# chongminggao/CIRS-codes

Measured on AMD Instinct MI355X. Metric: simulator env-steps/s (collect + PPO update in the timed region), KuaishouEnv, higher is better.
Workload: dtype f32 (policy/tracker; rollout on the fp32 MFMA, PPO head products fp32-accurate from two fp16 pieces per operand (3 f16 MFMAs per product), fp32 accumulate) + f64 (env rewards, GAE)

## Files before the change

cirs-codes_amd/csrc/ppo.hip:

```cpp
#include "internal.h"
#include "optim.h"
#include "bf16x6.h"
#include "small_gemm.h"
#include "permutation.h"
#include "policy_kernels.h"

namespace cirs {
typedef float f32x4 __attribute__((ext_vector_type(4)));


constexpr int kBwdWaves = 4;
__host__ __device__ inline int n_row_blocks_of(int n_pad) { return (n_pad / kTileM + kBwdWaves - 1) / kBwdWaves; }
__host__ __device__ inline size_t dwa_slab_stride(int I) { return (((size_t)I * 64 + I) + 3) & ~(size_t)3; }
__host__ __device__ inline int n_dwa_slabs_of(int n_pad) { return n_row_blocks_of(n_pad); }

struct PpoLayout {
    long w1, b1, w2, b2, wa, ba, wc, bc, total, trunk;
};
__host__ __device__ inline PpoLayout ppo_layout(int I, int S) {
    PpoLayout L;
    L.w1 = 0; L.b1 = L.w1 + (long)kH * S; L.w2 = L.b1 + kH; L.b2 = L.w2 + (long)kH * kH;
    L.trunk = L.b2 + kH;
    L.wa = L.trunk; L.ba = L.wa + (long)I * kH; L.wc = L.ba + I; L.bc = L.wc + kH; L.total = L.bc + 1;
    return L;
// ... 527 lines not shown
constexpr int kTStride = 36;
constexpr int kRSize = kTileN * kH + 2 * kTileN;
constexpr int kRowB = 144, kColB = 80;
constexpr int kRPlaneB = kTileN * kRowB, kCPlaneB = kH * kColB;
constexpr int kWBufB = 3 * kRPlaneB + 3 * kCPlaneB;

#ifdef CIRS_HEAD_PROF
__device__ unsigned long long g_step_prof[64];
#define CIRS_PSTAMP(COND, K) do { if ((COND) && threadIdx.x == 0) g_step_prof[K] = __builtin_amdgcn_s_memtime(); } while (0)
#else
#define CIRS_PSTAMP(COND, K) do { } while (0)
#endif
#ifdef CIRS_HEAD_PROF
__device__ unsigned long long g_head_prof[64];
#define CIRS_HSTAMP(K) do { if (blockIdx.x == 0 && blockIdx.y == 0 && threadIdx.x == 0 && it == 2) g_head_prof[K] = __builtin_amdgcn_s_memtime(); } while (0)
#define CIRS_TSTAMP(B, K) do { if ((int)blockIdx.x == (B) && threadIdx.x == 0) g_head_prof[K] = __builtin_amdgcn_s_memtime(); } while (0)
#define CIRS_SSTAMP(K) do { if (blockIdx.x == 0 && blockIdx.y == 0 && threadIdx.x == 0) g_head_prof[K] = __builtin_amdgcn_s_memtime(); } while (0)
#else
#define CIRS_HSTAMP(K) do { } while (0)
#define CIRS_TSTAMP(B, K) do { } while (0)
#define CIRS_SSTAMP(K) do { } while (0)
#endif
template <bool kZout>
__global__ __launch_bounds__(256, 2) void head_stats_kernel(int I, int mb, int n_pad, int tiles_per_chunk,
                                                            const uint4* __restrict__ planes, const float* __restrict__ ba,
                                                            const uint4* __restrict__ h2z, ActorPartialView pv,
                                                            const int32_t* __restrict__ act_rows, float* __restrict__ za_out,
                                                            float4* __restrict__ zslab) {
    __shared__ __attribute__((aligned(16))) unsigned char sW[2][3 * kRPlaneB];
    __shared__ __attribute__((aligned(16))) float sB[2][kTileN];
    const int tid = threadIdx.x;
    CIRS_SSTAMP(40);
    const int lane = tid & 63, wv = tid >> 6;
    const int hi = lane >> 5, lo = lane & 31;
// ... 119 lines not shown
            run_s = run_s * fa + osum * fb;
            run_t = run_t * fa + ot * fb;
            run_m = mn;
        }
    }
    if (hi == 0) {
        const size_t po = (size_t)chunk * n_pad + jr;
        pv.score[po] = run_t; pv.m[po] = run_m; pv.s[po] = run_s;
    }
    if (za_have) za_out[jr] = za_val;
}



struct HeadMergeArgs { cirs_ppo_cfg cfg; cirs_ppo_batch b; const int32_t* idx; int mb_norm, n_schunks; ActorPartialView pv; };
template <bool kEnt, bool kMerge, bool kZin>
__global__ __launch_bounds__(kBwdWaves * 64, 1) void head_bwd_fused_kernel(int I, int mb, int n_pad, int tiles_per_chunk,
                                                                         const uint4* __restrict__ planes,
                                                                         const float* __restrict__ ba, MbView v,
                                                                         float* __restrict__ dwap, HeadMergeArgs ma) {
    constexpr int kThreads = kBwdWaves * 64;
    static_assert(kThreads == 256, "the plane staging maps one 16-byte unit per thread and plane");
    constexpr int kCOff = kZin ? 0 : 3 * kRPlaneB;
    __shared__ __attribute__((aligned(16))) unsigned char sW[2][kCOff + 3 * kCPlaneB];
    __shared__ __attribute__((aligned(16))) float sB[2][kTileN];
    __shared__ __attribute__((aligned(16))) float sT[kBwdWaves][kTileN * kTStride];
    __shared__ __attribute__((aligned(16))) float sR[2][kBwdWaves][kRSize];
    const int tid = threadIdx.x;
    CIRS_SSTAMP(30);
    if (blockIdx.x == 0 && blockIdx.y == 0) {
        v.sync[tid] = 0;
        if (tid < kSyncInts - 256) v.sync[256 + tid] = 0;
    }
    const int lane = tid & 63, wv = tid >> 6;
    const int hi = lane >> 5, lo = lane & 31;
    const int row0 = (blockIdx.y * kBwdWaves + wv) * kTileM;
    const bool wave_ok = row0 < n_pad;
    const int chunk = blockIdx.x;
    if (chunk * tiles_per_chunk * kTileN >= I) return;
    const int jr = wave_ok ? row0 + lo : 0;
    const float kLog2e = 1.4426950408889634f, kLn2 = 0.6931471805599453f;
    const int act = v.act[jr];
    HPl hz[4];
    HPl hb[2][2];
    {
        const size_t tb = (size_t)((wave_ok ? row0 : 0) >> 5) * 12 * 64 + lane;
        const uint4* zp = v.h2z + tb;
        const uint4* bp = v.h2b + tb;
        if (!kZin) {
#pragma unroll
            for (int s4 = 0; s4 < 4; ++s4) {
                HPL_SET(hz[s4], zp[(3 * s4) * 64], zp[(3 * s4 + 2) * 64]);
            }
        }
#pragma unroll
        for (int c = 0; c < 2; ++c)
#pragma unroll
            for (int t = 0; t < 2; ++t) {
                HPL_SET(hb[c][t], bp[(3 * (2 * c + t)) * 64], bp[(3 * (2 * c + t) + 2) * 64]);
            }
    }
    const bool row_ok = wave_ok && jr < mb;
    f32x16 dh0, dh1;
#pragma unroll
    for (int r = 0; r < 16; ++r) { dh0[r] = 0.f; dh1[r] = 0.f; }
    float ent = 0.f;
    const float eps = 1.1920928955078125e-7f;
    const float kLogEps = -15.942385152878742f, kLog1mEps = -1.1920929665620834e-7f;
    if (!wave_ok) {
        for (int q = lane; q < kRSize; q += 64) { sR[0][wv][q] = 0.f; sR[1][wv][q] = 0.f; }
    }

    const int first_tile = chunk * tiles_per_chunk * kTileN;
    const int n_tiles = max(0, min(tiles_per_chunk, (I - first_tile + kTileN - 1) / kTileN));
    const int dst_r = (tid >> 3) * kRowB + (tid & 7) * 16;
    const int dst_c = kCOff + (tid >> 2) * kColB + (tid & 3) * 16;
    uint4 gr0, gr2, gc0, gc2;
    float gb = 0.f;
#define CIRS_ISSUE(TILE0)                                                                                  \
    do {                                                                                                   \
        const uint4* src_ = planes + (size_t)((TILE0) / kTileN) * kPlaneTileU4 + tid;                      \
        if (!kZin) { gr0 = src_[0]; gr2 = src_[512]; }                                                     \
        gc0 = src_[768]; gc2 = src_[1280];                                                                 \
        if (!kZin && tid < kTileN) gb = ((TILE0) + tid) < I ? kScZ * ba[(TILE0) + tid] : 0.f;    \
    } while (0)
#define CIRS_COMMIT(BUF)                                                                                   \
    do {                                                                                                   \
        unsigned char* base_ = sW[BUF];                                                                    \
        if (!kZin) {                                                                                       \
            *reinterpret_cast<uint4*>(base_ + dst_r) = gr0;                                                \
            *reinterpret_cast<uint4*>(base_ + 2 * kRPlaneB + dst_r) = gr2;                                 \
        }                                                                                                  \
        *reinterpret_cast<uint4*>(base_ + dst_c) = gc0;                                                    \
        \
        *reinterpret_cast<uint4*>(base_ + 2 * kCPlaneB + dst_c) = gc2;                                     \
        if (!kZin && tid < kTileN) sB[BUF][tid] = gb;                                                      \
    } while (0)
    const float4* zsl = v.zslab + ((size_t)(first_tile / kTileN) * (n_pad / kTileM) + (wave_ok ? row0 / kTileM : 0)) * kZTileF4 + lane;
    const size_t zstep = (size_t)(n_pad / kTileM) * kZTileF4;
    float4 zn[4];
    if (kZin) {
#pragma unroll
        for (int q = 0; q < 4; ++q) zn[q] = zsl[q * 64];
    }
    if (n_tiles > 0) CIRS_ISSUE(first_tile);
    float lse, c_logp, c_ent, h_ent;
    if (!kMerge) {
        lse = v.lse[jr]; c_logp = v.c_logp[jr]; c_ent = kEnt ? v.c_ent[jr] : 0.f; h_ent = kEnt ? v.h_ent[jr] : 0.f;
    } else {
        const bool real = wave_ok && jr < mb;
        const int jc = real ? jr : 0;
        const float za = v.za[jc], adv = v.adv[jc], lpo = v.adv[n_pad + jc], ret = v.adv[2 * (size_t)n_pad + jc], vs = v.adv[3 * (size_t)n_pad + jc],
                    val = v.value[jc];
        const float red0 = v.red[0], red1 = v.red[1];
        const int nsc = ma.n_schunks;
        const float* __restrict__ pm_ = ma.pv.m + jc;
        const float* __restrict__ ps_ = ma.pv.s + jc;
        const float* __restrict__ pt_ = ma.pv.score + jc;
        float M = -INFINITY, ssum = 0.f, tsum = 0.f;
        const bool need_t = kEnt || blockIdx.x == 0;
// ... 34 lines not shown
        ssum += __shfl_xor(ssum, 32, CIRS_WAVE);
        tsum += __shfl_xor(tsum, 32, CIRS_WAVE);
        const float lse_r = M + __logf(ssum);
        const RowTerms rt = ppo_row_terms(ma.cfg, za, lse_r, tsum / ssum, lpo, adv, red0, red1, val, vs, ret, 1.0f / (float)ma.mb_norm);
        lse = real ? lse_r : 1e30f;
        c_logp = real ? rt.c_logp : 0.f;
        c_ent = (kEnt && real) ? rt.c_ent : 0.f;
        h_ent = (kEnt && real) ? rt.h_ent : 0.f;
        if (blockIdx.x == 0 && hi == 0 && wave_ok) {
            v.dvalue[jr] = real ? rt.dvalue : 0.f;
            v.clip_row[jr] = real ? rt.clip_row : 0.f;
            v.vf_row[jr] = real ? rt.vf_row : 0.f;
            v.h_ent[jr] = real ? rt.h_ent : 0.f;
        }
    }
    float dz_scale = 1.0f, dz_inv = 1.0f;
    __shared__ float s_cmax[kBwdWaves];
    {
        const float cm = wave_max_f32_dpp(fabsf(c_logp) + 16.0f * fabsf(c_ent));
        if (lane == 0) s_cmax[wv] = cm;
    }
    CIRS_SSTAMP(31);
    if (n_tiles > 0) CIRS_COMMIT(0);
    __syncthreads();
    {
        float cm = s_cmax[0];
#pragma unroll
        for (int q = 1; q < kBwdWaves; ++q) cm = fmaxf(cm, s_cmax[q]);
        int ex = 0;
        if (cm > 0.f) { (void)frexpf(cm, &ex); ex = max(ex, -80); dz_scale = ldexpf(1.0f, 14 - ex); dz_inv = ldexpf(1.0f, ex - 14); }
        c_logp *= dz_scale; c_ent *= dz_scale;
    }
    const float nlse2 = -(lse * kLog2e), ncl = -c_logp;
    CIRS_SSTAMP(32);
    float* slab = dwap + (size_t)blockIdx.y * dwa_slab_stride(I);
    constexpr int kRedQ = (kTileN * kH / 4) / kThreads;
    const float dw_unscale = dz_inv * (1.0f / kScH2), dh_unscale = dz_inv * (1.0f / kScWa);
    struct RedRegs { f32x4 t[kRedQ][kBwdWaves]; float b[kBwdWaves]; };
    auto reduce_load = [&](int rb, RedRegs& rg) {
#pragma unroll
        for (int q = 0; q < kRedQ; ++q)
#pragma unroll
            for (int w2 = 0; w2 < kBwdWaves; ++w2) rg.t[q][w2] = reinterpret_cast<const f32x4*>(sR[rb][w2])[tid + kThreads * q];
        if (wv == 0) {
#pragma unroll
            for (int w2 = 0; w2 < kBwdWaves; ++w2) rg.b[w2] = sR[rb][w2][kTileN * kH + lo] + sR[rb][w2][kTileN * kH + kTileN + lo];
        }
    };
    auto reduce_store = [&](const RedRegs& rg, int t0) {
        const bool full = t0 + kTileN <= I;
#pragma unroll
        for (int q = 0; q < kRedQ; ++q) {
            const int f = tid + kThreads * q;
            f32x4 t = rg.t[q][0];
#pragma unroll
            for (int w2 = 1; w2 < kBwdWaves; ++w2) t += rg.t[q][w2];
            t *= dw_unscale;
            if (full || t0 + (f >> 4) < I) *reinterpret_cast<f32x4*>(slab + (size_t)t0 * kH + 4 * f) = t;
        }
        if (wv == 0) {
            float t = rg.b[0];
#pragma unroll
            for (int w2 = 1; w2 < kBwdWaves; ++w2) t += rg.b[w2];
            if (hi == 0 && (full || t0 + lo < I)) slab[(size_t)I * kH + t0 + lo] = t * dz_inv;
        }
    };
    auto reduce_tile = [&](int rb, int t0) { RedRegs rg; reduce_load(rb, rg); reduce_store(rg, t0); };
    for (int it = 0; it < n_tiles; ++it) {
        const int buf = it & 1;
        const int tile0 = first_tile + it * kTileN;
        CIRS_HSTAMP(0);
        if (it + 1 < n_tiles) CIRS_ISSUE(tile0 + kTileN);
        f32x16 dw0, dw1;
        float db = 0.f;
        if (!wave_ok) {
            if (it + 1 < n_tiles) CIRS_COMMIT(buf ^ 1);
            if (it > 0) reduce_tile(buf ^ 1, tile0 - kTileN);
        }
        if (wave_ok) {
            const unsigned char* tw = sW[buf];
            HPl cb[2][2];
            f32x16 acc;
            RedRegs rg;
            if (kZin) {
#pragma unroll
                for (int q = 0; q < 4; ++q) { acc[4 * q] = zn[q].x; acc[4 * q + 1] = zn[q].y; acc[4 * q + 2] = zn[q].z; acc[4 * q + 3] = zn[q].w; }
                const float4* zp = zsl + (size_t)min(it + 1, n_tiles - 1) * zstep;
#pragma unroll
                for (int q = 0; q < 4; ++q) zn[q] = zp[q * 64];
                CIRS_HSTAMP(1);
            } else {
                HPl za[4];
#pragma unroll
                for (int s4 = 0; s4 < 4; ++s4) {
                    const unsigned char* ap = tw + lo * kRowB + (16 * s4 + 8 * hi) * 2;
                    HPL_SET(za[s4], *reinterpret_cast<const uint4*>(ap), *reinterpret_cast<const uint4*>(ap + 2 * kRPlaneB));
                }
                f32x16 acc1, acc2;
#pragma unroll
                for (int r = 0; r < 16; ++r) { acc[r] = sB[buf][acc_row(r, hi)]; acc1[r] = 0.f; acc2[r] = 0.f; }
                CIRS_HSTAMP(1);
                hmfma_split2(za[0], hz[0], za[1], hz[1], acc, acc1, acc2);
                if (it > 0) reduce_load(buf ^ 1, rg);
                hmfma_split2(za[2], hz[2], za[3], hz[3], acc, acc1, acc2);
#pragma unroll
                for (int r = 0; r < 16; ++r) acc[r] += acc1[r] + acc2[r];
                if (it > 0) reduce_store(rg, tile0 - kTileN);
            }
#pragma unroll
            for (int t = 0; t < 2; ++t)
#pragma unroll
                for (int c = 0; c < 2; ++c) {
                    const unsigned char* bp = tw + kCOff + (32 * c + lo) * kColB + (16 * t + 8 * hi) * 2;
                    HPL_SET(cb[c][t], *reinterpret_cast<const uint4*>(bp), *reinterpret_cast<const uint4*>(bp + 2 * kCPlaneB));
                }
            CIRS_HSTAMP(2);
            float* tt = sT[wv];
            f32x16 tk;
            float pmax = 0.f, elo = 0.f;
            f32x2_b elo2 = {0.f, 0.f};
            const float kTEps = -23.0f;
            const bool last_tile = tile0 + kTileN > I;
#pragma unroll
            for (int r = 0; r < 16; r += 2) {
                const float t0 = __builtin_fmaf(acc[r], kLog2e * kScZi, nlse2), t1 = __builtin_fmaf(acc[r + 1], kLog2e * kScZi, nlse2);
                const float p0 = __builtin_amdgcn_exp2f(t0), p1 = __builtin_amdgcn_exp2f(t1);
                tk[r] = t0; tk[r + 1] = t1;
                pmax = __builtin_fmaxf(__builtin_fmaxf(pmax, p0), p1);
                if (!last_tile) {
                    const f32x2_b d2 = f32x2_b{kTEps, kTEps} - f32x2_b{t0, t1};
                    const f32x2_b w2 = {__builtin_fmaxf(d2.x, 0.f), __builtin_fmaxf(d2.y, 0.f)};
                    elo2 = f32x2_b{p0, p1} * w2 + elo2;
                }
                if (kEnt) {
                    acc[r] = __builtin_fmaf(c_ent * p0, __builtin_fmaf(t0, kLn2, h_ent), ncl * p0);
                    acc[r + 1] = __builtin_fmaf(c_ent * p1, __builtin_fmaf(t1, kLn2, h_ent), ncl * p1);
                } else {
// ... 14 lines not shown
                }
            }
            ent -= kLn2 * (elo + (elo2.x + elo2.y));
            CIRS_HSTAMP(3);
#pragma unroll
            for (int r = 0; r < 16; ++r) tt[acc_row(r, hi) * kTStride + lo] = acc[r];
            if (__any(row_ok && pmax > 1.0f - eps)) {
#pragma unroll
                for (int r = 0; r < 16; ++r) {
                    const float p = __builtin_amdgcn_exp2f(tk[r]);
                    const bool ok = row_ok && (!last_tile || tile0 + acc_row(r, hi) < I);
                    ent -= (ok && p > 1.0f - eps) ? p * (kLog1mEps - tk[r] * kLn2) : 0.f;
                }
            }
            CIRS_HSTAMP(4);
            __builtin_amdgcn_fence(__ATOMIC_RELEASE, "wavefront");
            __builtin_amdgcn_wave_barrier();
            __builtin_amdgcn_fence(__ATOMIC_ACQUIRE, "wavefront");
            f32x16 dzt;
#pragma unroll
            for (int g = 0; g < 4; ++g) {
                const float4 t4 = *reinterpret_cast<const float4*>(&tt[lo * kTStride + 8 * g + 4 * hi]);
                dzt[4 * g] = t4.x; dzt[4 * g + 1] = t4.y; dzt[4 * g + 2] = t4.z; dzt[4 * g + 3] = t4.w;
            }
            if (it + 1 < n_tiles) CIRS_COMMIT(buf ^ 1);
            {
                const HPl a0 = hsplit8(acc, 0), a1 = hsplit8(acc, 8);
                if (kZin && it > 0) reduce_load(buf ^ 1, rg);
                hmfma_pair(a0, cb[0][0], cb[1][0], dh0, dh1);
                hmfma_pair(a1, cb[0][1], cb[1][1], dh0, dh1);
                if (kZin && it > 0) reduce_store(rg, tile0 - kTileN);
            }
            CIRS_HSTAMP(5);
            CIRS_HSTAMP(6);
#pragma unroll
            for (int r = 0; r < 16; ++r) { dw0[r] = 0.f; dw1[r] = 0.f; db += dzt[r]; }
            {
                const HPl b0 = hsplit8(dzt, 0), b1 = hsplit8(dzt, 8);
                hmfma_pair(b0, hb[0][0], hb[1][0], dw0, dw1);
                hmfma_pair(b1, hb[0][1], hb[1][1], dw0, dw1);
            }
        }
        CIRS_HSTAMP(7);
        if (wave_ok) {
            float* rr = sR[buf][wv];
#pragma unroll
// ... 26 lines not shown
    CIRS_SSTAMP(35);
}
typedef void (*HeadBwdFn)(int, int, int, int, const uint4*, const float*, MbView, float*, HeadMergeArgs);
__host__ inline HeadBwdFn head_bwd_fn(bool ent, bool merge, bool zin) {
    switch ((ent ? 4 : 0) | (merge ? 2 : 0) | (zin ? 1 : 0)) {
    case 0: return head_bwd_fused_kernel<false, false, false>;
    case 1: return head_bwd_fused_kernel<false, false, true>;
    case 2: return head_bwd_fused_kernel<false, true, false>;
    case 3: return head_bwd_fused_kernel<false, true, true>;
    case 4: return head_bwd_fused_kernel<true, false, false>;
    case 5: return head_bwd_fused_kernel<true, false, true>;
    case 6: return head_bwd_fused_kernel<true, true, false>;
    default: return head_bwd_fused_kernel<true, true, true>;
    }
}
__host__ inline bool head_recompute_env() {
    const char* e = getenv("CIRS_PPO_HEAD_RECOMPUTE");
    return e && atoi(e) != 0;
}

constexpr int kNormBlocks = 256;
constexpr int kWaSumBlocks = 176;
__device__ __forceinline__ void wa_slab_sum_block(float* __restrict__ g, long wa_beg, long wa_len, const float* __restrict__ dwap,
                                                  long slab_stride, int n_slabs, int b, float* __restrict__ partial_out, float* sh) {
    const int tid = threadIdx.x;
    float acc = 0.f;
    const long n4 = wa_len >> 2;
    for (long q4 = b * 1024L + tid; q4 < n4; q4 += (long)kWaSumBlocks * 1024) {
        const long q4b = q4 + 512;
        const bool has_b = q4b < n4;
// ... 1227 lines not shown
    const int n_item_tiles = cdiv(I, kTileN);
    const int tpc_s = head_tiles_per_chunk(n_item_tiles, n_slabs, 2);
    const int n_schunks = cdiv(n_item_tiles, tpc_s);
    const auto stats_fn = r.head_recompute ? head_stats_kernel<false> : head_stats_kernel<true>;
    CIRS_PROF_LAUNCH(2, r.s, hipLaunchKernelGGL(stats_fn, dim3(n_schunks, n_slabs), dim3(256), 0, r.s, I, mb, n_pad, tpc_s,
                                                (const uint4*)v.wa_planes, r.w.ba, (const uint4*)v.h2z, pv, (const int32_t*)v.act, v.za, v.zslab));
    CIRS_CHECK_LAUNCH("head_stats_kernel");
    const HeadMergeArgs hma{*r.cfg, *r.batch, st.idx, st.mb_norm, n_schunks, pv};
    if (r.merge_launch) {
        hipLaunchKernelGGL(head_stats_merge_kernel, dim3(cdiv(n_pad, 4)), dim3(256), 0, r.s, *r.cfg, *r.batch, st.idx, mb, st.mb_norm, n_pad, n_schunks,
                           r.n_env, pv, r.w.wa, r.w.ba, v, (const float*)nullptr, 0);
        CIRS_CHECK_LAUNCH("head_stats_merge_kernel");
    }
    const int tpc = head_tiles_per_chunk(n_item_tiles, n_slabs, 1);
    const int n_bchunks = cdiv(n_item_tiles, tpc);
    const dim3 bgrid((n_bchunks + 7) & ~7, n_slabs), bblock(kBwdWaves * 64);
    const HeadBwdFn bwd_fn = head_bwd_fn(r.cfg->ent_coef != 0.f, !r.merge_launch, !r.head_recompute);
    CIRS_PROF_LAUNCH(1, r.s, hipLaunchKernelGGL(bwd_fn, bgrid, bblock, 0, r.s, I, mb, n_pad, tpc, (const uint4*)v.wa_planes, (const float*)r.w.ba, v, v.dwap, hma));
    CIRS_CHECK_LAUNCH("head_bwd_fused_kernel");
    if (with_dh2_sum) {
        hipLaunchKernelGGL(dh2_sum_kernel, dim3(n_pad * (kH / 4) / 64 + cdiv(n_pad, 64)), dim3(64), 0, r.s, mb, n_pad, n_bchunks, v);
        CIRS_CHECK_LAUNCH("dh2_sum_kernel");
    }
    *n_bchunks_out = n_bchunks;
    return CIRS_OK;
}
static cirs::DwJobs trunk_dw_jobs(const PpoRun& r, int n_pad) {
    using namespace cirs;
    const MbView& v = r.v;
    DwJobs jobs{};
    jobs.n = 3;
// ... 294 lines not shown
        CIRS_CHECK_LAUNCH("head_tp_fold_kernel");
        return CIRS_OK;
    }
    if (phase == 2) {
        CIRS_REQUIRE(stats_all, "stats_all is null");
        ActorPartialView pa;
        pa.m = const_cast<float*>(stats_all); pa.s = pa.m + (size_t)world * n_pad; pa.score = pa.s + (size_t)world * n_pad;
        pa.idx = nullptr; pa.z = nullptr;
        const float* za = pa.score + (size_t)world * n_pad;
        hipLaunchKernelGGL(head_stats_merge_kernel, dim3(cdiv(n_pad, 4)), dim3(256), 0, s, *cfg, *batch, idx, (int)mb, (int)mb, n_pad, (int)world,
                           (int)n_env, pa, (const float*)nullptr, (const float*)nullptr, v, za, (int)item_base);
        CIRS_CHECK_LAUNCH("head_stats_merge_kernel");
        const int tpc = head_tiles_per_chunk(n_item_tiles, n_slabs, 1);
        const int n_bchunks = cdiv(n_item_tiles, tpc);
        const HeadMergeArgs no_merge{};
        hipLaunchKernelGGL(head_bwd_fn(cfg->ent_coef != 0.f, false, !head_recompute_env()), dim3((n_bchunks + 7) & ~7, n_slabs), dim3(kBwdWaves * 64), 0, s, I,
                           (int)mb, n_pad, tpc, (const uint4*)v.wa_planes, (const float*)w.ba, v, v.dwap, no_merge);
        CIRS_CHECK_LAUNCH("head_bwd_fused_kernel");
        CIRS_HIP(hipMemsetAsync(red_slots, 0, sizeof(float) * (size_t)world * kWaSumBlocks, s));
        hipLaunchKernelGGL(dh2_sum_kernel, dim3(n_pad * (kH / 4) / 64 + cdiv(n_pad, 64)), dim3(64), 0, s, (int)mb, n_pad, n_bchunks, v, red_dh2, red_ent);
        CIRS_CHECK_LAUNCH("dh2_sum_kernel");
        hipLaunchKernelGGL(wa_slab_sum_kernel, dim3(kWaSumBlocks), dim3(512), 0, s, grads, (long)L.wa, seg, (const float*)v.dwap,
                           (long)dwa_slab_stride(I), n_slabs, red_slots + (size_t)rank * kWaSumBlocks);
        CIRS_CHECK_LAUNCH("wa_slab_sum_kernel");
        return CIRS_OK;
    }
    CIRS_REQUIRE(loss_out, "loss_out is null");
    hipLaunchKernelGGL(tp_post_kernel, dim3(cdiv(n_pad, 256)), dim3(256), 0, s, (int)mb, n_pad, (int)world, (const float*)red_ent,
                       (const float*)red_slots, v);
    CIRS_CHECK_LAUNCH("tp_post_kernel");
    DwJobs jobs;
// ... 60 lines not shown
```

Before: 5.558 million.

## Split head backward kernel into producer and consumer wave roles for the zin path

For the default zin path, the head backward kernel now launches twice as many waves. Role-A waves compute softmax gradients and the dh MFMAs, while role-B waves stage weight planes into LDS, load h2 pieces and reduce the dW partials, using double-buffered sT and sR. This is meant to overlap the plane staging and slab reduction with the MFMA and exp work that was previously serialized within each wave. The cost is more LDS, a different block size, and extra cross-role synchronization; the recompute path keeps the old single-role kernel.

```diff
diff --git a/cirs-codes_amd/csrc/ppo.hip b/cirs-codes_amd/csrc/ppo.hip
--- a/cirs-codes_amd/csrc/ppo.hip
+++ b/cirs-codes_amd/csrc/ppo.hip
@@ -565,10 +565,12 @@
 #ifdef CIRS_HEAD_PROF
 __device__ unsigned long long g_head_prof[64];
 #define CIRS_HSTAMP(K) do { if (blockIdx.x == 0 && blockIdx.y == 0 && threadIdx.x == 0 && it == 2) g_head_prof[K] = __builtin_amdgcn_s_memtime(); } while (0)
+#define CIRS_HSTAMPB(K) do { if (blockIdx.x == 0 && blockIdx.y == 0 && threadIdx.x == 256 && it == 3) g_head_prof[K] = __builtin_amdgcn_s_memtime(); } while (0)
 #define CIRS_TSTAMP(B, K) do { if ((int)blockIdx.x == (B) && threadIdx.x == 0) g_head_prof[K] = __builtin_amdgcn_s_memtime(); } while (0)
 #define CIRS_SSTAMP(K) do { if (blockIdx.x == 0 && blockIdx.y == 0 && threadIdx.x == 0) g_head_prof[K] = __builtin_amdgcn_s_memtime(); } while (0)
 #else
 #define CIRS_HSTAMP(K) do { } while (0)
+#define CIRS_HSTAMPB(K) do { } while (0)
 #define CIRS_TSTAMP(B, K) do { } while (0)
 #define CIRS_SSTAMP(K) do { } while (0)
 #endif
@@ -718,96 +720,9 @@
 
 
 struct HeadMergeArgs { cirs_ppo_cfg cfg; cirs_ppo_batch b; const int32_t* idx; int mb_norm, n_schunks; ActorPartialView pv; };
-template <bool kEnt, bool kMerge, bool kZin>
-__global__ __launch_bounds__(kBwdWaves * 64, 1) void head_bwd_fused_kernel(int I, int mb, int n_pad, int tiles_per_chunk,
-                                                                         const uint4* __restrict__ planes,
-                                                                         const float* __restrict__ ba, MbView v,
-                                                                         float* __restrict__ dwap, HeadMergeArgs ma) {
-    constexpr int kThreads = kBwdWaves * 64;
-    static_assert(kThreads == 256, "the plane staging maps one 16-byte unit per thread and plane");
-    constexpr int kCOff = kZin ? 0 : 3 * kRPlaneB;
-    __shared__ __attribute__((aligned(16))) unsigned char sW[2][kCOff + 3 * kCPlaneB];
-    __shared__ __attribute__((aligned(16))) float sB[2][kTileN];
-    __shared__ __attribute__((aligned(16))) float sT[kBwdWaves][kTileN * kTStride];
-    __shared__ __attribute__((aligned(16))) float sR[2][kBwdWaves][kRSize];
-    const int tid = threadIdx.x;
-    CIRS_SSTAMP(30);
-    if (blockIdx.x == 0 && blockIdx.y == 0) {
-        v.sync[tid] = 0;
-        if (tid < kSyncInts - 256) v.sync[256 + tid] = 0;
-    }
-    const int lane = tid & 63, wv = tid >> 6;
-    const int hi = lane >> 5, lo = lane & 31;
-    const int row0 = (blockIdx.y * kBwdWaves + wv) * kTileM;
-    const bool wave_ok = row0 < n_pad;
-    const int chunk = blockIdx.x;
-    if (chunk * tiles_per_chunk * kTileN >= I) return;
-    const int jr = wave_ok ? row0 + lo : 0;
-    const float kLog2e = 1.4426950408889634f, kLn2 = 0.6931471805599453f;
-    const int act = v.act[jr];
-    HPl hz[4];
-    HPl hb[2][2];
-    {
-        const size_t tb = (size_t)((wave_ok ? row0 : 0) >> 5) * 12 * 64 + lane;
-        const uint4* zp = v.h2z + tb;
-        const uint4* bp = v.h2b + tb;
-        if (!kZin) {
-#pragma unroll
-            for (int s4 = 0; s4 < 4; ++s4) {
-                HPL_SET(hz[s4], zp[(3 * s4) * 64], zp[(3 * s4 + 2) * 64]);
-            }
-        }
-#pragma unroll
-        for (int c = 0; c < 2; ++c)
-#pragma unroll
-            for (int t = 0; t < 2; ++t) {
-                HPL_SET(hb[c][t], bp[(3 * (2 * c + t)) * 64], bp[(3 * (2 * c + t) + 2) * 64]);
-            }
-    }
-    const bool row_ok = wave_ok && jr < mb;
-    f32x16 dh0, dh1;
-#pragma unroll
-    for (int r = 0; r < 16; ++r) { dh0[r] = 0.f; dh1[r] = 0.f; }
-    float ent = 0.f;
-    const float eps = 1.1920928955078125e-7f;
-    const float kLogEps = -15.942385152878742f, kLog1mEps = -1.1920929665620834e-7f;
-    if (!wave_ok) {
-        for (int q = lane; q < kRSize; q += 64) { sR[0][wv][q] = 0.f; sR[1][wv][q] = 0.f; }
-    }
-
-    const int first_tile = chunk * tiles_per_chunk * kTileN;
-    const int n_tiles = max(0, min(tiles_per_chunk, (I - first_tile + kTileN - 1) / kTileN));
-    const int dst_r = (tid >> 3) * kRowB + (tid & 7) * 16;
-    const int dst_c = kCOff + (tid >> 2) * kColB + (tid & 3) * 16;
-    uint4 gr0, gr2, gc0, gc2;
-    float gb = 0.f;
-#define CIRS_ISSUE(TILE0)                                                                                  \
-    do {                                                                                                   \
-        const uint4* src_ = planes + (size_t)((TILE0) / kTileN) * kPlaneTileU4 + tid;                      \
-        if (!kZin) { gr0 = src_[0]; gr2 = src_[512]; }                                                     \
-        gc0 = src_[768]; gc2 = src_[1280];                                                                 \
-        if (!kZin && tid < kTileN) gb = ((TILE0) + tid) < I ? kScZ * ba[(TILE0) + tid] : 0.f;    \
-    } while (0)
-#define CIRS_COMMIT(BUF)                                                                                   \
-    do {                                                                                                   \
-        unsigned char* base_ = sW[BUF];                                                                    \
-        if (!kZin) {                                                                                       \
-            *reinterpret_cast<uint4*>(base_ + dst_r) = gr0;                                                \
-            *reinterpret_cast<uint4*>(base_ + 2 * kRPlaneB + dst_r) = gr2;                                 \
-        }                                                                                                  \
-        *reinterpret_cast<uint4*>(base_ + dst_c) = gc0;                                                    \
-        \
-        *reinterpret_cast<uint4*>(base_ + 2 * kCPlaneB + dst_c) = gc2;                                     \
-        if (!kZin && tid < kTileN) sB[BUF][tid] = gb;                                                      \
-    } while (0)
-    const float4* zsl = v.zslab + ((size_t)(first_tile / kTileN) * (n_pad / kTileM) + (wave_ok ? row0 / kTileM : 0)) * kZTileF4 + lane;
-    const size_t zstep = (size_t)(n_pad / kTileM) * kZTileF4;
-    float4 zn[4];
-    if (kZin) {
-#pragma unroll
-        for (int q = 0; q < 4; ++q) zn[q] = zsl[q * 64];
-    }
-    if (n_tiles > 0) CIRS_ISSUE(first_tile);
+struct HeadRowCoef { float lse, c_logp, c_ent, h_ent; };
+template <bool kEnt, bool kMerge>
+__device__ __forceinline__ HeadRowCoef head_row_coef(const MbView& v, const HeadMergeArgs& ma, int n_pad, int mb, bool wave_ok, int jr, int hi) {
     float lse, c_logp, c_ent, h_ent;
     if (!kMerge) {
         lse = v.lse[jr]; c_logp = v.c_logp[jr]; c_ent = kEnt ? v.c_ent[jr] : 0.f; h_ent = kEnt ? v.h_ent[jr] : 0.f;
@@ -872,15 +787,83 @@
             v.h_ent[jr] = real ? rt.h_ent : 0.f;
         }
     }
-    float dz_scale = 1.0f, dz_inv = 1.0f;
+    return HeadRowCoef{lse, c_logp, c_ent, h_ent};
+}
+constexpr int kBwdRoleThreads = 2 * kBwdWaves * 64;
+template <bool kEnt, bool kMerge>
+__device__ __forceinline__ void head_bwd_roles(int I, int mb, int n_pad, int tiles_per_chunk, const uint4* __restrict__ planes, const MbView& v,
+                                               float* __restrict__ dwap, const HeadMergeArgs& ma) {
+    constexpr int kStage = kBwdWaves * 64;
+    static_assert(kStage == 256, "the plane staging maps one 16-byte unit per thread and plane");
+    static_assert(kSyncInts <= kBwdRoleThreads, "one thread per arrival flag");
+    __shared__ __attribute__((aligned(16))) unsigned char sW[2][3 * kCPlaneB];
+    __shared__ __attribute__((aligned(16))) float sT[2][kBwdWaves][kTileN * kTStride];
+    __shared__ __attribute__((aligned(16))) float sR[2][kBwdWaves][kRSize];
     __shared__ float s_cmax[kBwdWaves];
-    {
+    static_assert(sizeof(sW) + sizeof(sT) + sizeof(sR) + sizeof(s_cmax) <= 160 * 1024, "LDS of one CU");
+    const int tid = threadIdx.x;
+    CIRS_SSTAMP(30);
+    if (blockIdx.x == 0 && blockIdx.y == 0 && tid < kSyncInts) v.sync[tid] = 0;
+    const int lane = tid & 63, wid = __builtin_amdgcn_readfirstlane(tid >> 6);
+    const bool role_b = wid >= kBwdWaves;
+    const int wv = wid & (kBwdWaves - 1), btid = tid & (kStage - 1);
+    const int hi = lane >> 5, lo = lane & 31;
+    const int row0 = (blockIdx.y * kBwdWaves + wv) * kTileM;
+    const bool wave_ok = row0 < n_pad;
+    const int chunk = blockIdx.x;
+    if (chunk * tiles_per_chunk * kTileN >= I) return;
+    const int jr = wave_ok ? row0 + lo : 0;
+    const bool row_ok = wave_ok && jr < mb;
+    const float kLog2e = 1.4426950408889634f, kLn2 = 0.6931471805599453f;
+    const float eps = 1.1920928955078125e-7f;
+    const float kLog1mEps = -1.1920929665620834e-7f;
+    const int first_tile = chunk * tiles_per_chunk * kTileN;
+    const int n_tiles = min(tiles_per_chunk, (I - first_tile + kTileN - 1) / kTileN);
+    const int dst_c = (btid >> 2) * kColB + (btid & 3) * 16;
+    uint4 gc0, gc2;
+#define CIRS_ISSUE(TILE0)                                                                                  \
+    do {                                                                                                   \
+        const uint4* src_ = planes + (size_t)((TILE0) / kTileN) * kPlaneTileU4 + btid;                     \
+        gc0 = src_[768]; gc2 = src_[1280];                                                                 \
+    } while (0)
+#define CIRS_COMMIT(BUF)                                                                                   \
+    do {                                                                                                   \
+        unsigned char* base_ = sW[BUF];                                                                    \
+        *reinterpret_cast<uint4*>(base_ + dst_c) = gc0;                                                    \
+        *reinterpret_cast<uint4*>(base_ + 2 * kCPlaneB + dst_c) = gc2;                                     \
+    } while (0)
+    const float4* zsl = v.zslab + ((size_t)(first_tile / kTileN) * (n_pad / kTileM) + (wave_ok ? row0 / kTileM : 0)) * kZTileF4 + lane;
+    const size_t zstep = (size_t)(n_pad / kTileM) * kZTileF4;
+    float4 zn[4];
+    int act = 0;
+    float lse = 0.f, c_logp = 0.f, c_ent = 0.f, h_ent = 0.f;
+    HPl hb[2][2];
+    if (!role_b) {
+        act = v.act[jr];
+#pragma unroll
+        for (int q = 0; q < 4; ++q) zn[q] = zsl[q * 64];
+        const HeadRowCoef rc = head_row_coef<kEnt, kMerge>(v, ma, n_pad, mb, wave_ok, jr, hi);
+        lse = rc.lse; c_logp = rc.c_logp; c_ent = rc.c_ent; h_ent = rc.h_ent;
         const float cm = wave_max_f32_dpp(fabsf(c_logp) + 16.0f * fabsf(c_ent));
         if (lane == 0) s_cmax[wv] = cm;
+    } else {
+        CIRS_ISSUE(first_tile);
+        const uint4* bp = v.h2b + (size_t)((wave_ok ? row0 : 0) >> 5) * 12 * 64 + lane;
+#pragma unroll
+        for (int c = 0; c < 2; ++c)
+#pragma unroll
+            for (int t = 0; t < 2; ++t) {
+                HPL_SET(hb[c][t], bp[(3 * (2 * c + t)) * 64], bp[(3 * (2 * c + t) + 2) * 64]);
+            }
+        if (!wave_ok) {
+            for (int q = lane; q < kRSize; q += 64) { sR[0][wv][q] = 0.f; sR[1][wv][q] = 0.f; }
+        }
+        CIRS_COMMIT(0);
     }
     CIRS_SSTAMP(31);
-    if (n_tiles > 0) CIRS_COMMIT(0);
     __syncthreads();
+    CIRS_SSTAMP(32);
+    float dz_scale = 1.0f, dz_inv = 1.0f;
     {
         float cm = s_cmax[0];
 #pragma unroll
@@ -889,96 +872,43 @@
         if (cm > 0.f) { (void)frexpf(cm, &ex); ex = max(ex, -80); dz_scale = ldexpf(1.0f, 14 - ex); dz_inv = ldexpf(1.0f, ex - 14); }
         c_logp *= dz_scale; c_ent *= dz_scale;
     }
-    const float nlse2 = -(lse * kLog2e), ncl = -c_logp;
-    CIRS_SSTAMP(32);
-    float* slab = dwap + (size_t)blockIdx.y * dwa_slab_stride(I);
-    constexpr int kRedQ = (kTileN * kH / 4) / kThreads;
     const float dw_unscale = dz_inv * (1.0f / kScH2), dh_unscale = dz_inv * (1.0f / kScWa);
-    struct RedRegs { f32x4 t[kRedQ][kBwdWaves]; float b[kBwdWaves]; };
-    auto reduce_load = [&](int rb, RedRegs& rg) {
-#pragma unroll
-        for (int q = 0; q < kRedQ; ++q)
-#pragma unroll
-            for (int w2 = 0; w2 < kBwdWaves; ++w2) rg.t[q][w2] = reinterpret_cast<const f32x4*>(sR[rb][w2])[tid + kThreads * q];
-        if (wv == 0) {
-#pragma unroll
-            for (int w2 = 0; w2 < kBwdWaves; ++w2) rg.b[w2] = sR[rb][w2][kTileN * kH + lo] + sR[rb][w2][kTileN * kH + kTileN + lo];
-        }
-    };
-    auto reduce_store = [&](const RedRegs& rg, int t0) {
-        const bool full = t0 + kTileN <= I;
-#pragma unroll
-        for (int q = 0; q < kRedQ; ++q) {
-            const int f = tid + kThreads * q;
-            f32x4 t = rg.t[q][0];
-#pragma unroll
-            for (int w2 = 1; w2 < kBwdWaves; ++w2) t += rg.t[q][w2];
-            t *= dw_unscale;
-            if (full || t0 + (f >> 4) < I) *reinterpret_cast<f32x4*>(slab + (size_t)t0 * kH + 4 * f) = t;
-        }
-        if (wv == 0) {
-            float t = rg.b[0];
-#pragma unroll
-            for (int w2 = 1; w2 < kBwdWaves; ++w2) t += rg.b[w2];
-            if (hi == 0 && (full || t0 + lo < I)) slab[(size_t)I * kH + t0 + lo] = t * dz_inv;
-        }
-    };
-    auto reduce_tile = [&](int rb, int t0) { RedRegs rg; reduce_load(rb, rg); reduce_store(rg, t0); };
-    for (int it = 0; it < n_tiles; ++it) {
-        const int buf = it & 1;
-        const int tile0 = first_tile + it * kTileN;
-        CIRS_HSTAMP(0);
-        if (it + 1 < n_tiles) CIRS_ISSUE(tile0 + kTileN);
-        f32x16 dw0, dw1;
-        float db = 0.f;
-        if (!wave_ok) {
-            if (it + 1 < n_tiles) CIRS_COMMIT(buf ^ 1);
-            if (it > 0) reduce_tile(buf ^ 1, tile0 - kTileN);
-        }
-        if (wave_ok) {
+
+    if (!role_b) {
+        f32x16 dh0, dh1;
+#pragma unroll
+        for (int r = 0; r < 16; ++r) { dh0[r] = 0.f; dh1[r] = 0.f; }
+        float ent = 0.f;
+        const float nlse2 = -(lse * kLog2e), ncl = -c_logp;
+        auto a_tile = [&](auto last_c, int it) {
+            constexpr bool last_tile = decltype(last_c)::value;
+            const int buf = it & 1;
+            const int tile0 = first_tile + it * kTileN;
             const unsigned char* tw = sW[buf];
+            CIRS_HSTAMP(0);
             HPl cb[2][2];
             f32x16 acc;
-            RedRegs rg;
-            if (kZin) {
-#pragma unroll
-                for (int q = 0; q < 4; ++q) { acc[4 * q] = zn[q].x; acc[4 * q + 1] = zn[q].y; acc[4 * q + 2] = zn[q].z; acc[4 * q + 3] = zn[q].w; }
+#pragma unroll
+            for (int q = 0; q < 4; ++q) { acc[4 * q] = zn[q].x; acc[4 * q + 1] = zn[q].y; acc[4 * q + 2] = zn[q].z; acc[4 * q + 3] = zn[q].w; }
+            {
                 const float4* zp = zsl + (size_t)min(it + 1, n_tiles - 1) * zstep;
 #pragma unroll
                 for (int q = 0; q < 4; ++q) zn[q] = zp[q * 64];
-                CIRS_HSTAMP(1);
-            } else {
-                HPl za[4];
-#pragma unroll
-                for (int s4 = 0; s4 < 4; ++s4) {
-                    const unsigned char* ap = tw + lo * kRowB + (16 * s4 + 8 * hi) * 2;
-                    HPL_SET(za[s4], *reinterpret_cast<const uint4*>(ap), *reinterpret_cast<const uint4*>(ap + 2 * kRPlaneB));
-                }
-                f32x16 acc1, acc2;
-#pragma unroll
-                for (int r = 0; r < 16; ++r) { acc[r] = sB[buf][acc_row(r, hi)]; acc1[r] = 0.f; acc2[r] = 0.f; }
-                CIRS_HSTAMP(1);
-                hmfma_split2(za[0], hz[0], za[1], hz[1], acc, acc1, acc2);
-                if (it > 0) reduce_load(buf ^ 1, rg);
-                hmfma_split2(za[2], hz[2], za[3], hz[3], acc, acc1, acc2);
-#pragma unroll
-                for (int r = 0; r < 16; ++r) acc[r] += acc1[r] + acc2[r];
-                if (it > 0) reduce_store(rg, tile0 - kTileN);
-            }
+            }
+            CIRS_HSTAMP(1);
 #pragma unroll
             for (int t = 0; t < 2; ++t)
 #pragma unroll
                 for (int c = 0; c < 2; ++c) {
-                    const unsigned char* bp = tw + kCOff + (32 * c + lo) * kColB + (16 * t + 8 * hi) * 2;
+                    const unsigned char* bp = tw + (32 * c + lo) * kColB + (16 * t + 8 * hi) * 2;
                     HPL_SET(cb[c][t], *reinterpret_cast<const uint4*>(bp), *reinterpret_cast<const uint4*>(bp + 2 * kCPlaneB));
                 }
             CIRS_HSTAMP(2);
-            float* tt = sT[wv];
+            float* tt = sT[buf][wv];
             f32x16 tk;
             float pmax = 0.f, elo = 0.f;
             f32x2_b elo2 = {0.f, 0.f};
             const float kTEps = -23.0f;
-            const bool last_tile = tile0 + kTileN > I;
 #pragma unroll
             for (int r = 0; r < 16; r += 2) {
                 const float t0 = __builtin_fmaf(acc[r], kLog2e * kScZi, nlse2), t1 = __builtin_fmaf(acc[r + 1], kLog2e * kScZi, nlse2);
@@ -1023,6 +953,343 @@
                 }
             }
             CIRS_HSTAMP(4);
+            const HPl a0 = hsplit8(acc, 0), a1 = hsplit8(acc, 8);
+            hmfma_pair(a0, cb[0][0], cb[1][0], dh0, dh1);
+            hmfma_pair(a1, cb[0][1], cb[1][1], dh0, dh1);
+            CIRS_HSTAMP(5);
+        };
+        if (wave_ok) {
+            for (int it = 0; it + 1 < n_tiles; ++it) { a_tile(std::false_type{}, it); lds_barrier(); CIRS_HSTAMP(10); }
+            if (first_tile + n_tiles * kTileN > I) a_tile(std::true_type{}, n_tiles - 1);
+            else a_tile(std::false_type{}, n_tiles - 1);
+            lds_barrier();
+            lds_barrier();
+            CIRS_SSTAMP(33);
+            float* hslab = v.dh2p + (size_t)chunk * n_pad * kH;
+#pragma unroll
+            for (int r = 0; r < 16; ++r) {
+                const int row = row0 + acc_row(r, hi);
+                hslab[(size_t)row * kH + lo] = dh0[r] * dh_unscale;
+                hslab[(size_t)row * kH + 32 + lo] = dh1[r] * dh_unscale;
+            }
+            ent += __shfl_xor(ent, 32, CIRS_WAVE);
+            if (hi == 0) v.entp[(size_t)chunk * n_pad + jr] = ent;
+            CIRS_SSTAMP(35);
+        } else {
+            for (int it = 0; it <= n_tiles; ++it) lds_barrier();
+        }
+    } else {
+        float* slab = dwap + (size_t)blockIdx.y * dwa_slab_stride(I);
+        constexpr int kRedQ = (kTileN * kH / 4) / kStage;
+        struct RedRegs { f32x4 t[kRedQ][kBwdWaves]; float b[kBwdWaves]; };
+        auto reduce_load = [&](int rb, RedRegs& rg) {
+#pragma unroll
+            for (int q = 0; q < kRedQ; ++q)
+#pragma unroll
+                for (int w2 = 0; w2 < kBwdWaves; ++w2) rg.t[q][w2] = reinterpret_cast<const f32x4*>(sR[rb][w2])[btid + kStage * q];
+            if (wv == 0) {
+#pragma unroll
+                for (int w2 = 0; w2 < kBwdWaves; ++w2) rg.b[w2] = sR[rb][w2][kTileN * kH + lo] + sR[rb][w2][kTileN * kH + kTileN + lo];
+            }
+        };
+        auto reduce_store = [&](const RedRegs& rg, int t0) {
+            const bool full = t0 + kTileN <= I;
+#pragma unroll
+            for (int q = 0; q < kRedQ; ++q) {
+                const int f = btid + kStage * q;
+                f32x4 t = rg.t[q][0];
+#pragma unroll
+                for (int w2 = 1; w2 < kBwdWaves; ++w2) t += rg.t[q][w2];
+                t *= dw_unscale;
+                if (full || t0 + (f >> 4) < I) *reinterpret_cast<f32x4*>(slab + (size_t)t0 * kH + 4 * f) = t;
+            }
+            if (wv == 0) {
+                float t = rg.b[0];
+#pragma unroll
+                for (int w2 = 1; w2 < kBwdWaves; ++w2) t += rg.b[w2];
+                if (hi == 0 && (full || t0 + lo < I)) slab[(size_t)I * kH + t0 + lo] = t * dz_inv;
+            }
+        };
+        auto b_iter = [&](auto steady_c, int it) {
+            constexpr bool kSteady = decltype(steady_c)::value;
+            const bool issue = kSteady || it + 1 < n_tiles, mma = kSteady || it >= 1, red = kSteady || it >= 2;
+            CIRS_HSTAMPB(11);
+            if (issue) CIRS_ISSUE(first_tile + (it + 1) * kTileN);
+            const int pb = (it & 1) ^ 1;
+            const bool prod = wave_ok && mma;
+            f32x16 dzt;
+            if (prod) {
+                const float* tt = sT[pb][wv];
+#pragma unroll
+                for (int g = 0; g < 4; ++g) {
+                    const float4 t4 = *reinterpret_cast<const float4*>(&tt[lo * kTStride + 8 * g + 4 * hi]);
+                    dzt[4 * g] = t4.x; dzt[4 * g + 1] = t4.y; dzt[4 * g + 2] = t4.z; dzt[4 * g + 3] = t4.w;
+                }
+            }
+            RedRegs rg;
+            if (red) reduce_load(it & 1, rg);
+            CIRS_HSTAMPB(12);
+            f32x16 dw0, dw1;
+            float db = 0.f;
+            if (prod) {
+#pragma unroll
+                for (int r = 0; r < 16; ++r) { dw0[r] = 0.f; dw1[r] = 0.f; db += dzt[r]; }
+                const HPl b0 = hsplit8(dzt, 0), b1 = hsplit8(dzt, 8);
+                hmfma_pair(b0, hb[0][0], hb[1][0], dw0, dw1);
+                hmfma_pair(b1, hb[0][1], hb[1][1], dw0, dw1);
+            }
+            CIRS_HSTAMPB(13);
+            if (issue) CIRS_COMMIT(pb);
+            if (red) reduce_store(rg, first_tile + (it - 2) * kTileN);
+            CIRS_HSTAMPB(14);
+            if (prod) {
+                float* rr = sR[pb][wv];
+#pragma unroll
+                for (int r = 0; r < 16; ++r) {
+                    const int il = acc_row(r, hi);
+                    rr[il * kH + lo] = dw0[r];
+                    rr[il * kH + 32 + lo] = dw1[r];
+                }
+                rr[kTileN * kH + lane] = db;
+            }
+            CIRS_HSTAMPB(15);
+        };
+        for (int it = 0; it <= n_tiles; ++it) {
+            if (it >= 2 && it + 1 < n_tiles) b_iter(std::true_type{}, it);
+            else b_iter(std::false_type{}, it);
+            lds_barrier();
+        }
+        RedRegs rg;
+        reduce_load((n_tiles - 1) & 1, rg);
+        reduce_store(rg, first_tile + (n_tiles - 1) * kTileN);
+    }
+#undef CIRS_ISSUE
+#undef CIRS_COMMIT
+}
+template <bool kEnt, bool kMerge, bool kZin>
+__global__ __launch_bounds__(kZin ? kBwdRoleThreads : kBwdWaves * 64, 1) void head_bwd_fused_kernel(int I, int mb, int n_pad, int tiles_per_chunk,
+                                                                                                  const uint4* __restrict__ planes,
+                                                                                                  const float* __restrict__ ba, MbView v,
+                                                                                                  float* __restrict__ dwap, HeadMergeArgs ma) {
+    if constexpr (kZin) { head_bwd_roles<kEnt, kMerge>(I, mb, n_pad, tiles_per_chunk, planes, v, dwap, ma); return; }
+    constexpr int kThreads = kBwdWaves * 64;
+    static_assert(kThreads == 256, "the plane staging maps one 16-byte unit per thread and plane");
+    constexpr int kCOff = 3 * kRPlaneB;
+    __shared__ __attribute__((aligned(16))) unsigned char sW[2][kCOff + 3 * kCPlaneB];
+    __shared__ __attribute__((aligned(16))) float sB[2][kTileN];
+    __shared__ __attribute__((aligned(16))) float sT[kBwdWaves][kTileN * kTStride];
+    __shared__ __attribute__((aligned(16))) float sR[2][kBwdWaves][kRSize];
+    const int tid = threadIdx.x;
+    CIRS_SSTAMP(30);
+    if (blockIdx.x == 0 && blockIdx.y == 0) {
+        v.sync[tid] = 0;
+        if (tid < kSyncInts - 256) v.sync[256 + tid] = 0;
+    }
+    const int lane = tid & 63, wv = tid >> 6;
+    const int hi = lane >> 5, lo = lane & 31;
+    const int row0 = (blockIdx.y * kBwdWaves + wv) * kTileM;
+    const bool wave_ok = row0 < n_pad;
+    const int chunk = blockIdx.x;
+    if (chunk * tiles_per_chunk * kTileN >= I) return;
+    const int jr = wave_ok ? row0 + lo : 0;
+    const float kLog2e = 1.4426950408889634f, kLn2 = 0.6931471805599453f;
+    const int act = v.act[jr];
+    HPl hz[4];
+    HPl hb[2][2];
+    {
+        const size_t tb = (size_t)((wave_ok ? row0 : 0) >> 5) * 12 * 64 + lane;
+        const uint4* zp = v.h2z + tb;
+        const uint4* bp = v.h2b + tb;
+#pragma unroll
+        for (int s4 = 0; s4 < 4; ++s4) {
+            HPL_SET(hz[s4], zp[(3 * s4) * 64], zp[(3 * s4 + 2) * 64]);
+        }
+#pragma unroll
+        for (int c = 0; c < 2; ++c)
+#pragma unroll
+            for (int t = 0; t < 2; ++t) {
+                HPL_SET(hb[c][t], bp[(3 * (2 * c + t)) * 64], bp[(3 * (2 * c + t) + 2) * 64]);
+            }
+    }
+    const bool row_ok = wave_ok && jr < mb;
+    f32x16 dh0, dh1;
+#pragma unroll
+    for (int r = 0; r < 16; ++r) { dh0[r] = 0.f; dh1[r] = 0.f; }
+    float ent = 0.f;
+    const float eps = 1.1920928955078125e-7f;
+    const float kLogEps = -15.942385152878742f, kLog1mEps = -1.1920929665620834e-7f;
+    if (!wave_ok) {
+        for (int q = lane; q < kRSize; q += 64) { sR[0][wv][q] = 0.f; sR[1][wv][q] = 0.f; }
+    }
+
+    const int first_tile = chunk * tiles_per_chunk * kTileN;
+    const int n_tiles = max(0, min(tiles_per_chunk, (I - first_tile + kTileN - 1) / kTileN));
+    const int dst_r = (tid >> 3) * kRowB + (tid & 7) * 16;
+    const int dst_c = kCOff + (tid >> 2) * kColB + (tid & 3) * 16;
+    uint4 gr0, gr2, gc0, gc2;
+    float gb = 0.f;
+#define CIRS_ISSUE(TILE0)                                                                                  \
+    do {                                                                                                   \
+        const uint4* src_ = planes + (size_t)((TILE0) / kTileN) * kPlaneTileU4 + tid;                      \
+        gr0 = src_[0]; gr2 = src_[512];                                                                    \
+        gc0 = src_[768]; gc2 = src_[1280];                                                                 \
+        if (tid < kTileN) gb = ((TILE0) + tid) < I ? kScZ * ba[(TILE0) + tid] : 0.f;    \
+    } while (0)
+#define CIRS_COMMIT(BUF)                                                                                   \
+    do {                                                                                                   \
+        unsigned char* base_ = sW[BUF];                                                                    \
+        *reinterpret_cast<uint4*>(base_ + dst_r) = gr0;                                                    \
+        *reinterpret_cast<uint4*>(base_ + 2 * kRPlaneB + dst_r) = gr2;                                     \
+        *reinterpret_cast<uint4*>(base_ + dst_c) = gc0;                                                    \
+        \
+        *reinterpret_cast<uint4*>(base_ + 2 * kCPlaneB + dst_c) = gc2;                                     \
+        if (tid < kTileN) sB[BUF][tid] = gb;                                                      \
+    } while (0)
+    if (n_tiles > 0) CIRS_ISSUE(first_tile);
+    const HeadRowCoef rc = head_row_coef<kEnt, kMerge>(v, ma, n_pad, mb, wave_ok, jr, hi);
+    float lse = rc.lse, c_logp = rc.c_logp, c_ent = rc.c_ent, h_ent = rc.h_ent;
+    float dz_scale = 1.0f, dz_inv = 1.0f;
+    __shared__ float s_cmax[kBwdWaves];
+    {
+        const float cm = wave_max_f32_dpp(fabsf(c_logp) + 16.0f * fabsf(c_ent));
+        if (lane == 0) s_cmax[wv] = cm;
+    }
+    CIRS_SSTAMP(31);
+    if (n_tiles > 0) CIRS_COMMIT(0);
+    __syncthreads();
+    {
+        float cm = s_cmax[0];
+#pragma unroll
+        for (int q = 1; q < kBwdWaves; ++q) cm = fmaxf(cm, s_cmax[q]);
+        int ex = 0;
+        if (cm > 0.f) { (void)frexpf(cm, &ex); ex = max(ex, -80); dz_scale = ldexpf(1.0f, 14 - ex); dz_inv = ldexpf(1.0f, ex - 14); }
+        c_logp *= dz_scale; c_ent *= dz_scale;
+    }
+    const float nlse2 = -(lse * kLog2e), ncl = -c_logp;
+    CIRS_SSTAMP(32);
+    float* slab = dwap + (size_t)blockIdx.y * dwa_slab_stride(I);
+    constexpr int kRedQ = (kTileN * kH / 4) / kThreads;
+    const float dw_unscale = dz_inv * (1.0f / kScH2), dh_unscale = dz_inv * (1.0f / kScWa);
+    struct RedRegs { f32x4 t[kRedQ][kBwdWaves]; float b[kBwdWaves]; };
+    auto reduce_load = [&](int rb, RedRegs& rg) {
+#pragma unroll
+        for (int q = 0; q < kRedQ; ++q)
+#pragma unroll
+            for (int w2 = 0; w2 < kBwdWaves; ++w2) rg.t[q][w2] = reinterpret_cast<const f32x4*>(sR[rb][w2])[tid + kThreads * q];
+        if (wv == 0) {
+#pragma unroll
+            for (int w2 = 0; w2 < kBwdWaves; ++w2) rg.b[w2] = sR[rb][w2][kTileN * kH + lo] + sR[rb][w2][kTileN * kH + kTileN + lo];
+        }
+    };
+    auto reduce_store = [&](const RedRegs& rg, int t0) {
+        const bool full = t0 + kTileN <= I;
+#pragma unroll
+        for (int q = 0; q < kRedQ; ++q) {
+            const int f = tid + kThreads * q;
+            f32x4 t = rg.t[q][0];
+#pragma unroll
+            for (int w2 = 1; w2 < kBwdWaves; ++w2) t += rg.t[q][w2];
+            t *= dw_unscale;
+            if (full || t0 + (f >> 4) < I) *reinterpret_cast<f32x4*>(slab + (size_t)t0 * kH + 4 * f) = t;
+        }
+        if (wv == 0) {
+            float t = rg.b[0];
+#pragma unroll
+            for (int w2 = 1; w2 < kBwdWaves; ++w2) t += rg.b[w2];
+            if (hi == 0 && (full || t0 + lo < I)) slab[(size_t)I * kH + t0 + lo] = t * dz_inv;
+        }
+    };
+    auto reduce_tile = [&](int rb, int t0) { RedRegs rg; reduce_load(rb, rg); reduce_store(rg, t0); };
+    for (int it = 0; it < n_tiles; ++it) {
+        const int buf = it & 1;
+        const int tile0 = first_tile + it * kTileN;
+        CIRS_HSTAMP(0);
+        if (it + 1 < n_tiles) CIRS_ISSUE(tile0 + kTileN);
+        f32x16 dw0, dw1;
+        float db = 0.f;
+        if (!wave_ok) {
+            if (it + 1 < n_tiles) CIRS_COMMIT(buf ^ 1);
+            if (it > 0) reduce_tile(buf ^ 1, tile0 - kTileN);
+        }
+        if (wave_ok) {
+            const unsigned char* tw = sW[buf];
+            HPl cb[2][2];
+            f32x16 acc;
+            RedRegs rg;
+            HPl za[4];
+#pragma unroll
+            for (int s4 = 0; s4 < 4; ++s4) {
+                const unsigned char* ap = tw + lo * kRowB + (16 * s4 + 8 * hi) * 2;
+                HPL_SET(za[s4], *reinterpret_cast<const uint4*>(ap), *reinterpret_cast<const uint4*>(ap + 2 * kRPlaneB));
+            }
+            f32x16 acc1, acc2;
+#pragma unroll
+            for (int r = 0; r < 16; ++r) { acc[r] = sB[buf][acc_row(r, hi)]; acc1[r] = 0.f; acc2[r] = 0.f; }
+            CIRS_HSTAMP(1);
+            hmfma_split2(za[0], hz[0], za[1], hz[1], acc, acc1, acc2);
+            if (it > 0) reduce_load(buf ^ 1, rg);
+            hmfma_split2(za[2], hz[2], za[3], hz[3], acc, acc1, acc2);
+#pragma unroll
+            for (int r = 0; r < 16; ++r) acc[r] += acc1[r] + acc2[r];
+            if (it > 0) reduce_store(rg, tile0 - kTileN);
+#pragma unroll
+            for (int t = 0; t < 2; ++t)
+#pragma unroll
+                for (int c = 0; c < 2; ++c) {
+                    const unsigned char* bp = tw + kCOff + (32 * c + lo) * kColB + (16 * t + 8 * hi) * 2;
+                    HPL_SET(cb[c][t], *reinterpret_cast<const uint4*>(bp), *reinterpret_cast<const uint4*>(bp + 2 * kCPlaneB));
+                }
+            CIRS_HSTAMP(2);
+            float* tt = sT[wv];
+            f32x16 tk;
+            float pmax = 0.f, elo = 0.f;
+            f32x2_b elo2 = {0.f, 0.f};
+            const float kTEps = -23.0f;
+            const bool last_tile = tile0 + kTileN > I;
+#pragma unroll
+            for (int r = 0; r < 16; r += 2) {
+                const float t0 = __builtin_fmaf(acc[r], kLog2e * kScZi, nlse2), t1 = __builtin_fmaf(acc[r + 1], kLog2e * kScZi, nlse2);
+                const float p0 = __builtin_amdgcn_exp2f(t0), p1 = __builtin_amdgcn_exp2f(t1);
+                tk[r] = t0; tk[r + 1] = t1;
+                pmax = __builtin_fmaxf(__builtin_fmaxf(pmax, p0), p1);
+                if (!last_tile) {
+                    const f32x2_b d2 = f32x2_b{kTEps, kTEps} - f32x2_b{t0, t1};
+                    const f32x2_b w2 = {__builtin_fmaxf(d2.x, 0.f), __builtin_fmaxf(d2.y, 0.f)};
+                    elo2 = f32x2_b{p0, p1} * w2 + elo2;
+                }
+                if (kEnt) {
+                    acc[r] = __builtin_fmaf(c_ent * p0, __builtin_fmaf(t0, kLn2, h_ent), ncl * p0);
+                    acc[r + 1] = __builtin_fmaf(c_ent * p1, __builtin_fmaf(t1, kLn2, h_ent), ncl * p1);
+                } else {
+                    acc[r] = ncl * p0; acc[r + 1] = ncl * p1;
+                }
+            }
+            if (__any(act >= tile0 && act < tile0 + kTileN)) {
+                const int rel = act - tile0 - 4 * hi;
+#pragma unroll
+                for (int r = 0; r < 16; ++r) acc[r] += (rel == (r & 3) + 8 * (r >> 2)) ? c_logp : 0.f;
+            }
+            if (last_tile) {
+#pragma unroll
+                for (int r = 0; r < 16; ++r) {
+                    const bool in = tile0 + acc_row(r, hi) < I;
+                    acc[r] = in ? acc[r] : 0.f;
+                    elo += in ? __builtin_amdgcn_exp2f(tk[r]) * __builtin_fmaxf(kTEps - tk[r], 0.f) : 0.f;
+                }
+            }
+            ent -= kLn2 * (elo + (elo2.x + elo2.y));
+            CIRS_HSTAMP(3);
+#pragma unroll
+            for (int r = 0; r < 16; ++r) tt[acc_row(r, hi) * kTStride + lo] = acc[r];
+            if (__any(row_ok && pmax > 1.0f - eps)) {
+#pragma unroll
+                for (int r = 0; r < 16; ++r) {
+                    const float p = __builtin_amdgcn_exp2f(tk[r]);
+                    const bool ok = row_ok && (!last_tile || tile0 + acc_row(r, hi) < I);
+                    ent -= (ok && p > 1.0f - eps) ? p * (kLog1mEps - tk[r] * kLn2) : 0.f;
+                }
+            }
+            CIRS_HSTAMP(4);
             __builtin_amdgcn_fence(__ATOMIC_RELEASE, "wavefront");
             __builtin_amdgcn_wave_barrier();
             __builtin_amdgcn_fence(__ATOMIC_ACQUIRE, "wavefront");
@@ -1035,10 +1302,8 @@
             if (it + 1 < n_tiles) CIRS_COMMIT(buf ^ 1);
             {
                 const HPl a0 = hsplit8(acc, 0), a1 = hsplit8(acc, 8);
-                if (kZin && it > 0) reduce_load(buf ^ 1, rg);
                 hmfma_pair(a0, cb[0][0], cb[1][0], dh0, dh1);
                 hmfma_pair(a1, cb[0][1], cb[1][1], dh0, dh1);
-                if (kZin && it > 0) reduce_store(rg, tile0 - kTileN);
             }
             CIRS_HSTAMP(5);
             CIRS_HSTAMP(6);
@@ -1095,6 +1360,7 @@
     default: return head_bwd_fused_kernel<true, true, true>;
     }
 }
+__host__ inline int head_bwd_threads(bool zin) { return zin ? kBwdRoleThreads : kBwdWaves * 64; }
 __host__ inline bool head_recompute_env() {
     const char* e = getenv("CIRS_PPO_HEAD_RECOMPUTE");
     return e && atoi(e) != 0;
@@ -2352,7 +2618,7 @@
     }
     const int tpc = head_tiles_per_chunk(n_item_tiles, n_slabs, 1);
     const int n_bchunks = cdiv(n_item_tiles, tpc);
-    const dim3 bgrid((n_bchunks + 7) & ~7, n_slabs), bblock(kBwdWaves * 64);
+    const dim3 bgrid((n_bchunks + 7) & ~7, n_slabs), bblock(head_bwd_threads(!r.head_recompute));
     const HeadBwdFn bwd_fn = head_bwd_fn(r.cfg->ent_coef != 0.f, !r.merge_launch, !r.head_recompute);
     CIRS_PROF_LAUNCH(1, r.s, hipLaunchKernelGGL(bwd_fn, bgrid, bblock, 0, r.s, I, mb, n_pad, tpc, (const uint4*)v.wa_planes, (const float*)r.w.ba, v, v.dwap, hma));
     CIRS_CHECK_LAUNCH("head_bwd_fused_kernel");
@@ -2677,7 +2943,8 @@
         const int tpc = head_tiles_per_chunk(n_item_tiles, n_slabs, 1);
         const int n_bchunks = cdiv(n_item_tiles, tpc);
         const HeadMergeArgs no_merge{};
-        hipLaunchKernelGGL(head_bwd_fn(cfg->ent_coef != 0.f, false, !head_recompute_env()), dim3((n_bchunks + 7) & ~7, n_slabs), dim3(kBwdWaves * 64), 0, s, I,
+        const bool zin = !head_recompute_env();
+        hipLaunchKernelGGL(head_bwd_fn(cfg->ent_coef != 0.f, false, zin), dim3((n_bchunks + 7) & ~7, n_slabs), dim3(head_bwd_threads(zin)), 0, s, I,
                            (int)mb, n_pad, tpc, (const uint4*)v.wa_planes, (const float*)w.ba, v, v.dwap, no_merge);
         CIRS_CHECK_LAUNCH("head_bwd_fused_kernel");
         CIRS_HIP(hipMemsetAsync(red_slots, 0, sizeof(float) * (size_t)world * kWaSumBlocks, s));
```

Result: faster. 5.797 million (median of 6 runs) (+4.3%).
